# dselivanov/rsparse

Hardware: AMD Instinct MI355X
Metric: als_iterations_per_sec (higher is better)
Workload: dtype f32 (Gram products of rows > 512 / <= 32 non-zeros as 2 x fp16 / 3 x bf16 split terms of the fp32 operands, fp32 accumulate; everything else fp32); 1 GPU; WRMF implicit ALS, CG(3), synthetic 10000000x1000000, 500155883 nnz, rank 128, lambda 0.1; survey_config=3, feedback=implicit, n_items=1000000, nnz=500155883, rank=128, solver=conjugate_gradient, cg_steps=3, parallelism=rows sharded x1, factors replicated

## Files before the change

rsparse_amd/build.py:

```python
import subprocess
import sys
import time
from concurrent.futures import ThreadPoolExecutor
from pathlib import Path

PKG = Path(__file__).resolve().parent
CSRC = PKG / "csrc"
SRC = [CSRC / n for n in ("wrmf_kernels.hip", "wrmf_cgq.hip", "wrmf_cgp.hip", "wrmf_ne.hip", "wrmf_chol.hip", "wrmf_chol_wave.hip", "wrmf_chol_mf.hip", "wrmf_cg_mf.hip", "wrmf_chol_lr.hip",
                          "wrmf_topk.hip", "wrmf_topk_large.hip", "wrmf_similar.hip", "wrmf_metrics.hip", "wrmf_hits.hip", "wrmf_lists.hip", "wrmf_diversity.hip", "wrmf_mmr.hip", "wrmf_ranks.hip", "wrmf_score.hip", "wrmf_candidates.hip", "wrmf_sample.hip", "wrmf_sample_weighted.hip", "wrmf_split.hip", "wrmf_explain.hip", "wrmf_init.hip", "wrmf_ingest.hip", "wrmf_nnls.hip", "wrmf_bias.hip", "wrmf_lu.hip",
                          "wrmf_f64.hip", "wrmf_wide.hip", "wrmf_wide_cg.hip", "wrmf_ctx_kernels.hip", "wrmf_schedule.cpp", "wrmf_capi.cpp", "wrmf_f64_capi.cpp", "wrmf_ctx.cpp")]
HEADERS = [CSRC / "wrmf_chol_mf.attrs.csv", CSRC / "wrmf_mf.h", CSRC / "wrmf_internal.h", CSRC / "wrmf_capi_common.h", CSRC / "wrmf_schedule.h", CSRC / "wrmf_device.h", CSRC / "wrmf_sample_team.h", CSRC / "wrmf_wave.h", CSRC / "wrmf_ldlt.h", CSRC / "wrmf_f64.h", PKG.parent / "include" / "rsparse_wrmf_hip.h"]
DEPS = SRC + HEADERS
OUT = PKG / "lib" / "librsparse_wrmf_hip.so"
FLAGS = ["--offload-arch=gfx950", "-O3", "-std=c++17", "-fPIC"]


EXTRA_FLAGS = {n: ["-mllvm", "-forceattrs-csv-path=" + str(CSRC / "wrmf_chol_mf.attrs.csv"), "-fno-slp-vectorize"] for n in ("wrmf_chol_mf.hip", "wrmf_cg_mf.hip")}
AUDITED = {"wrmf_chol_mf.hip", "wrmf_cg_mf.hip"}
REG_LIMIT = {"wrmf_cg_mf.hip": 512}
NO_SPILL = {"wrmf_cgq.hip": ("14als_cgq_kernelILi128ELi24ELi4ELi4E",),
            "wrmf_explain.hip": ("14explain_kernelIfLi128E",),
            "wrmf_sample.hip": ("13sample_kernelILi64E", "13sample_kernelILi256E"),
            "wrmf_sample_weighted.hip": ("22sample_weighted_kernelILi64E", "22sample_weighted_kernelILi256E"),
            "wrmf_hits.hip": ("18hit_metrics_kernelILb0E", "18hit_metrics_kernelILb1E"),
            "wrmf_lists.hip": ("19list_metrics_kernelILb0E", "19list_metrics_kernelILb1E"),
            "wrmf_diversity.hip": ("21list_diversity_kernelI", "21item_inv_norms_kernelI"),
            "wrmf_mmr.hip": ("10mmr_kernelI",),
            "wrmf_split.hip": ("split_count_wave_kernel", "split_count_team_kernel", "split_write_wave_kernel", "split_write_team_kernel")}
RESOURCE_FLAG = "-Rpass-analysis=kernel-resource-usage"


def resource_violations(remarks, patterns, limit=256):
    import re
    rows, cur = [], None
    for line in remarks.splitlines():
        m = re.search(r"remark:\s+(.*?) \[-Rpass", line)
        if not m:
            continue
        t = m.group(1).strip()
        if t.startswith("Function Name:"):
            cur = {"name": t.split(":", 1)[1].strip()}
            rows.append(cur)
        elif ":" in t and cur is not None:
            k, v = t.rsplit(":", 1)
            cur[k.strip()] = v.strip()
    bad = []
    for pat in patterns:
        hit = [r for r in rows if pat in r["name"]]
        if not hit:
            bad.append((pat, "no such kernel in the compilation"))
        for r in hit:
            regs = int(r.get("VGPRs", "0")) + int(r.get("AGPRs", "0"))
            for key in ("VGPRs Spill", "ScratchSize [bytes/lane]"):
                if int(r.get(key, "0")):
                    bad.append((r["name"], "%s = %s" % (key, r[key])))
            if regs > limit:
                bad.append((r["name"], "%d vector registers" % regs))
    return bad


def audit_listing(src, extra, obj):
    sys.path.insert(0, str(PKG.parent / "tools" / "dbg"))
    import acc_audit
    lst = obj.with_suffix(".s")

    def listing(flags, floor):
        cmd = ["hipcc", *FLAGS, *flags, "-S", "--cuda-device-only", str(src), "-o", str(lst)]
        r = subprocess.run(cmd, stdout=subprocess.PIPE, stderr=subprocess.PIPE, text=True)
        if r.returncode != 0:
            raise RuntimeError("hipcc -S failed on %s:\n%s" % (src.name, r.stderr[-3000:]))
        acc, flight, _ = acc_audit.audit(str(lst), quiet=True, acc_floor=floor)
        return acc, flight, lst.read_text()
    acc, flight, text = listing(extra, 0)
    import re
    nfree = re.findall(r"\.amdhsa_kernel (\w+)[\s\S]*?\.amdhsa_next_free_vgpr (\d+)", text)
    limit = REG_LIMIT.get(src.name, 256)
    two_waves = bool(nfree) and all(int(v) <= limit for name, v in nfree if "_any" not in name)
    if acc == 0 and flight == 0 and two_waves:
        return
    print("  %s: audit of the two-waves-per-SIMD build failed (accumulator-file %d, in-flight %d, layout ok %s): rebuilding with -DMF_SAFE"
          % (src.name, acc, flight, two_waves), flush=True)
    safe = ["-DMF_SAFE"]
    cmd = ["hipcc", *FLAGS, *safe, "-c", str(src), "-o", str(obj)]
    r = subprocess.run(cmd, stdout=subprocess.PIPE, stderr=subprocess.PIPE, text=True)
    if r.returncode != 0:
        raise RuntimeError("hipcc failed on %s (MF_SAFE):\n%s" % (src.name, r.stderr[-3000:]))
    acc, flight, text = listing(safe, 96)
    if acc or flight:
        raise RuntimeError("%s: the MF_SAFE build fails the audit too (accumulator-file %d, in-flight %d)" % (src.name, acc, flight))


def build(force=False, verbose=False, out=None):
    out = Path(out) if out else OUT
    out.parent.mkdir(exist_ok=True)
    objdir = OUT.parent / "obj"
    objdir.mkdir(parents=True, exist_ok=True)
    src = [s for s in SRC if s.exists()]
    hdr_m = max(h.stat().st_mtime for h in HEADERS)
    todo, objs = [], []
    for s in src:
        o = objdir / (s.stem + ".o")
        objs.append(o)
        if force or not o.exists() or o.stat().st_mtime < max(s.stat().st_mtime, hdr_m):
            todo.append((s, o))
    if not todo and out.exists() and all(out.stat().st_mtime >= o.stat().st_mtime for o in objs):
        return out

    def compile_one(so):
        s, o = so
        t0 = time.time()
        extra = EXTRA_FLAGS.get(s.name, [])
        guard = NO_SPILL.get(s.name)
        cmd = ["hipcc", *FLAGS, *extra, *([RESOURCE_FLAG] if guard else []), "-c", str(s), "-o", str(o)]
        r = subprocess.run(cmd, stdout=subprocess.PIPE, stderr=subprocess.PIPE, text=True)
        if r.returncode != 0:
            raise RuntimeError("hipcc failed on %s:\n%s" % (s.name, r.stderr[-6000:]))
        if guard:
            bad = resource_violations(r.stderr, guard)
            if bad:
                o.unlink()
                raise RuntimeError("%s: kernels that must not spill do:\n%s" % (s.name, "\n".join("  %s: %s" % b for b in bad)))
        if s.name in AUDITED:
            audit_listing(s, extra, o)
        if verbose:
            print("  %-20s %.1f s" % (s.name, time.time() - t0), flush=True)

    with ThreadPoolExecutor(max_workers=8) as ex:
        list(ex.map(compile_one, todo))
    cmd = ["hipcc", "--offload-arch=gfx950", "-fPIC", "-shared", *map(str, objs), "-ldl", "-lpthread", "-o", str(out)]
    subprocess.check_call(cmd)
    return out


if __name__ == "__main__":
    argv = sys.argv[1:]
    outp = argv[argv.index("--out") + 1] if "--out" in argv else None
    t0 = time.time()
    print(build(force="--force" in argv, verbose=True, out=outp), "%.1f s" % (time.time() - t0))
```

rsparse_amd/csrc/wrmf_kernels.hip:

```cpp
#include "wrmf_internal.h"
#include "wrmf_device.h"

namespace rsparse_hip {
namespace {

using namespace dev;

template <int KP, int T, int W, bool IMPLICIT>
struct CgSmem {
  static constexpr int LDT = Geo<KP>::LDT;
  static constexpr size_t gram_floats = IMPLICIT ? (size_t)KP * KP : 0;
  static constexpr size_t tile_floats = (size_t)W * T * LDT;
  static constexpr size_t vec_floats = (size_t)W * KP;
  static constexpr size_t red_floats = (size_t)2 * W * KP + 2 * W;
  static constexpr size_t short_bytes = (gram_floats + tile_floats + vec_floats) * 4 + 16;
  static constexpr size_t long_bytes = (gram_floats + tile_floats + vec_floats + red_floats) * 4 + 16;
};

template <int KP, int W>
__device__ __forceinline__ void load_gram_lds(float* sG, const float* __restrict__ G, int k, int tid) {
  for (int e = tid; e < KP * KP; e += W * 64) {
    const int r = e / KP, c = e % KP;
    sG[e] = (r < k && c < k) ? G[(size_t)r * k + c] : 0.f;
  }
}

template <int KP, int T, int W, bool IMPLICIT, bool VEC>
__global__ __launch_bounds__(W * 64) void als_cg_short_kernel(AlsArgs a) {
  constexpr int EPL = Geo<KP>::EPL, LDT = Geo<KP>::LDT;
  extern __shared__ __attribute__((aligned(16))) char smem[];
  float* sG = reinterpret_cast<float*>(smem);
  float* sTiles = sG + CgSmem<KP, T, W, IMPLICIT>::gram_floats;
  float* sVecs = sTiles + CgSmem<KP, T, W, IMPLICIT>::tile_floats;
  int* sCtr = reinterpret_cast<int*>(sVecs + CgSmem<KP, T, W, IMPLICIT>::vec_floats);

  const int tid = threadIdx.x, lane = tid & 63, wv = rfl(tid >> 6);
  const int k = a.k;
  if constexpr (IMPLICIT) load_gram_lds<KP, W>(sG, a.XtX, k, tid);
  for (int e = tid; e < (int)(CgSmem<KP, T, W, IMPLICIT>::tile_floats + CgSmem<KP, T, W, IMPLICIT>::vec_floats);
       e += W * 64)
    sTiles[e] = 0.f;
  if (tid == 0) *sCtr = 0;
  __syncthreads();

  float* tile = sTiles + wv * T * LDT;
  float* vec = sVecs + wv * KP;
  const int row0 = blockIdx.x * kRowsPerWGShort;
  const int row_end = min(a.n_cols, row0 + kRowsPerWGShort);
  const int e0 = lane * EPL;
  const bool active = e0 < KP;
  const int jl = lane % T;
  double wloss = 0.0;
  const bool gb = IMPLICIT && a.gbias != 0.f;
  const float gbias = gb ? a.gbias : 0.f, ltgt = gb ? a.loss_tgt_const : 1.f;

  while (true) {
    int rr = 0;
    if (lane == 0) rr = atomicAdd(sCtr, 1);
    const int row = row0 + rfl(rr);
    if (row >= row_end) break;
    const int p1 = rfl(a.col_ptrs[row]), p2 = rfl(a.col_ptrs[row + 1]);
    const int cnt = p2 - p1;
    if (cnt > T) continue;
    float* yrow = a.Y + (size_t)row * k;
    if (cnt <= 0 && !gb) {
      for (int e = lane; e < k; e += 64) yrow[e] = 0.f;
      continue;
    }
    const bool jvalid = jl < cnt;
    const int myidx = jvalid ? a.row_idx[p1 + jl] : 0;
    const float c = jvalid ? a.vals[p1 + jl] : 0.f;
    wave_sync();
    gather_chunk<KP, T, VEC>(a.X, k, myidx, cnt, tile, lane);

    float x[EPL], r[EPL], p[EPL], ap[EPL];
#pragma unroll
    for (int u = 0; u < EPL; u++) x[u] = (active && e0 + u < k) ? yrow[e0 + u] : 0.f;
    const float lam_use =
        IMPLICIT ? 0.f : (float)(a.lambda_loss * (a.dynamic_lambda ? (double)(float)cnt : 1.0));

    put_vec<KP>(vec, x, lane, active);
    wave_sync();
    float t = tile_dot<KP, T>(tile, vec, lane);
    float wgt = jvalid ? (IMPLICIT ? c - (c - 1.f) * (t + gbias) : c - t) : 0.f;
#pragma unroll
    for (int u = 0; u < EPL; u++) r[u] = 0.f;
    tile_axpy<KP>(tile, wgt, cnt, lane, active, r);
    if constexpr (IMPLICIT) {
      gram_mv<KP>(sG, vec, 0, KP, lane, active, -1.f, r);
      if (gb) {
#pragma unroll
        for (int u = 0; u < EPL; u++) r[u] += (active && e0 + u < k) ? a.rhs_init[e0 + u] : 0.f;
      }
    } else {
#pragma unroll
      for (int u = 0; u < EPL; u++) r[u] -= lam_use * x[u];
    }
    float rs = 0.f;
#pragma unroll
    for (int u = 0; u < EPL; u++) { p[u] = r[u]; rs = fmaf(r[u], r[u], rs); }
    float rsold = wave_sum(rs);

    for (int it = 0; it < a.cg_steps; ++it) {
      wave_sync();
      put_vec<KP>(vec, p, lane, active);
      wave_sync();
      t = tile_dot<KP, T>(tile, vec, lane);
      wgt = jvalid ? (IMPLICIT ? (c - 1.f) * t : t) : 0.f;
#pragma unroll
      for (int u = 0; u < EPL; u++) ap[u] = 0.f;
      tile_axpy<KP>(tile, wgt, cnt, lane, active, ap);
      if constexpr (IMPLICIT) {
        gram_mv<KP>(sG, vec, 0, KP, lane, active, 1.f, ap);
      } else {
#pragma unroll
        for (int u = 0; u < EPL; u++) ap[u] = fmaf(lam_use, p[u], ap[u]);
      }
      float pap = 0.f;
#pragma unroll
      for (int u = 0; u < EPL; u++) pap = fmaf(p[u], ap[u], pap);
      pap = wave_sum(pap);
      const float alpha = (float)((double)rsold / (double)pap);
      rs = 0.f;
#pragma unroll
      for (int u = 0; u < EPL; u++) {
        x[u] = fmaf(alpha, p[u], x[u]);
        r[u] = fmaf(-alpha, ap[u], r[u]);
        rs = fmaf(r[u], r[u], rs);
      }
      const float rsnew = wave_sum(rs);
      if (rsnew < kCgTol) break;
      const float beta = (float)((double)rsnew / (double)rsold);
#pragma unroll
      for (int u = 0; u < EPL; u++) p[u] = fmaf(p[u], beta, r[u]);
      rsold = rsnew;
    }

    wave_sync();
    put_vec<KP>(vec, x, lane, active);
    wave_sync();
    t = tile_dot<KP, T>(tile, vec, lane);
    const float d = IMPLICIT ? ltgt - t : c - t;
    const float lj = (jvalid && lane < T) ? (IMPLICIT ? c * d * d : d * d) : 0.f;
    const float rl = wave_sum(lj);
    float xx = 0.f;
#pragma unroll
    for (int u = 0; u < EPL; u++) xx = fmaf(x[u], x[u], xx);
    xx = wave_sum(xx);
    wloss += IMPLICIT ? (double)rl + a.lambda_loss * (double)xx : (double)(rl + lam_use * xx);
#pragma unroll
    for (int u = 0; u < EPL; u++)
      if (active && e0 + u < k) yrow[e0 + u] = x[u];
  }
  if (lane == 0) a.loss_partials[(size_t)blockIdx.x * W + wv] = wloss;
}

template <int KP, int T, int W, bool IMPLICIT, bool VEC>
__global__ __launch_bounds__(W * 64) void als_cg_long_kernel(AlsArgs a, size_t loss_slot0) {
  constexpr int EPL = Geo<KP>::EPL, LDT = Geo<KP>::LDT;
  static_assert(KP % (4 * W) == 0, "Gramian k-range must split evenly over the waves");
  extern __shared__ __attribute__((aligned(16))) char smem[];
  float* sG = reinterpret_cast<float*>(smem);
  float* sTiles = sG + CgSmem<KP, T, W, IMPLICIT>::gram_floats;
  float* sVecs = sTiles + CgSmem<KP, T, W, IMPLICIT>::tile_floats;
  float* sRed = sVecs + CgSmem<KP, T, W, IMPLICIT>::vec_floats;
  float* sRedL = sRed + 2 * W * KP;

  const int tid = threadIdx.x, lane = tid & 63, wv = rfl(tid >> 6);
  const int k = a.k;
  if constexpr (IMPLICIT) load_gram_lds<KP, W>(sG, a.XtX, k, tid);
  for (int e = tid; e < (int)(CgSmem<KP, T, W, IMPLICIT>::tile_floats + CgSmem<KP, T, W, IMPLICIT>::vec_floats +
                              CgSmem<KP, T, W, IMPLICIT>::red_floats);
       e += W * 64)
    sTiles[e] = 0.f;
  __syncthreads();

  float* tile = sTiles + wv * T * LDT;
  float* vec = sVecs + wv * KP;
  const int e0 = lane * EPL;
  const bool active = e0 < KP;
  const int jl = lane % T;
  int buf = 0;
  double wloss = 0.0;
  const bool gb = IMPLICIT && a.gbias != 0.f;
  const float gbias = gb ? a.gbias : 0.f, ltgt = gb ? a.loss_tgt_const : 1.f;

  for (int li = blockIdx.x; li < a.n_long; li += gridDim.x) {
    const int row = rfl(a.long_rows[li]);
    const int p1 = rfl(a.col_ptrs[row]), p2 = rfl(a.col_ptrs[row + 1]);
    const int cnt = p2 - p1;
    const int nchunks = (cnt + T - 1) / T;
    const bool resident = nchunks <= W;
    float* yrow = a.Y + (size_t)row * k;
    const float lam_use =
        IMPLICIT ? 0.f : (float)(a.lambda_loss * (a.dynamic_lambda ? (double)(float)cnt : 1.0));

    int ccnt = 0, cidx = 0;
    float cval = 0.f;
    if (resident && wv < nchunks) {
      const int base = p1 + wv * T;
      ccnt = min(T, p2 - base);
      cidx = jl < ccnt ? a.row_idx[base + jl] : 0;
      cval = jl < ccnt ? a.vals[base + jl] : 0.f;
      wave_sync();
      gather_chunk<KP, T, VEC>(a.X, k, cidx, ccnt, tile, lane);
      wave_sync();
    }

    float x[EPL], r[EPL], p[EPL], ap[EPL];
#pragma unroll
    for (int u = 0; u < EPL; u++) x[u] = (active && e0 + u < k) ? yrow[e0 + u] : 0.f;

    auto sweep = [&](const float(&v)[EPL], const int mode, float(&out)[EPL], float& loss_out) {
      wave_sync();
      put_vec<KP>(vec, v, lane, active);
      wave_sync();
      float acc[EPL];
#pragma unroll
      for (int u = 0; u < EPL; u++) acc[u] = 0.f;
      float lacc = 0.f;
      for (int ch = wv; ch < nchunks; ch += W) {
        if (!resident) {
          const int base = p1 + ch * T;
          ccnt = min(T, p2 - base);
          cidx = jl < ccnt ? a.row_idx[base + jl] : 0;
          cval = jl < ccnt ? a.vals[base + jl] : 0.f;
          wave_sync();
          gather_chunk<KP, T, VEC>(a.X, k, cidx, ccnt, tile, lane);
          wave_sync();
        }
        const bool jvalid = jl < ccnt;
        const float t = tile_dot<KP, T>(tile, vec, lane);
        if (mode == 2) {
          const float d = IMPLICIT ? ltgt - t : cval - t;
          lacc += (jvalid && lane < T) ? (IMPLICIT ? cval * d * d : d * d) : 0.f;
        } else {
          float wgt;
          if (mode == 0) wgt = IMPLICIT ? cval - (cval - 1.f) * (t + gbias) : cval - t;
          else wgt = IMPLICIT ? (cval - 1.f) * t : t;
          wgt = jvalid ? wgt : 0.f;
          tile_axpy<KP>(tile, wgt, ccnt, lane, active, acc);
        }
      }
      float* red = sRed + buf * W * KP;
      if (mode == 2) {
        lacc = wave_sum(lacc);
        if (lane == 0) sRedL[buf * W + wv] = lacc;
      } else {
        if constexpr (IMPLICIT)
          gram_mv<KP>(sG, vec, wv * (KP / W), (wv + 1) * (KP / W), lane, active, mode == 0 ? -1.f : 1.f, acc);
        put_vec<KP>(red + wv * KP, acc, lane, active);
      }
      __syncthreads();
      if (mode == 2) {
        float s = 0.f;
#pragma unroll
        for (int w2 = 0; w2 < W; w2++) s += sRedL[buf * W + w2];
        loss_out = s;
      } else {
#pragma unroll
        for (int u = 0; u < EPL; u++) out[u] = 0.f;
#pragma unroll
        for (int w2 = 0; w2 < W; w2++) {
          if constexpr (EPL == 2) {
            const float2 q = *reinterpret_cast<const float2*>(red + w2 * KP + lane * 2);
            out[0] += q.x;
            out[1] += q.y;
          } else {
            out[0] += active ? red[w2 * KP + lane] : 0.f;
          }
        }
        if constexpr (!IMPLICIT) {
#pragma unroll
          for (int u = 0; u < EPL; u++) out[u] = fmaf(mode == 0 ? -lam_use : lam_use, v[u], out[u]);
        } else if (gb && mode == 0) {
#pragma unroll
          for (int u = 0; u < EPL; u++) out[u] += (active && e0 + u < k) ? a.rhs_init[e0 + u] : 0.f;
        }
      }
      buf ^= 1;
    };

    float dummy = 0.f;
    sweep(x, 0, r, dummy);
    float rs = 0.f;
#pragma unroll
    for (int u = 0; u < EPL; u++) { p[u] = r[u]; rs = fmaf(r[u], r[u], rs); }
    float rsold = wave_sum(rs);
    for (int it = 0; it < a.cg_steps; ++it) {
      sweep(p, 1, ap, dummy);
      float pap = 0.f;
#pragma unroll
      for (int u = 0; u < EPL; u++) pap = fmaf(p[u], ap[u], pap);
      pap = wave_sum(pap);
      const float alpha = (float)((double)rsold / (double)pap);
      rs = 0.f;
#pragma unroll
      for (int u = 0; u < EPL; u++) {
        x[u] = fmaf(alpha, p[u], x[u]);
        r[u] = fmaf(-alpha, ap[u], r[u]);
        rs = fmaf(r[u], r[u], rs);
      }
      const float rsnew = wave_sum(rs);
      if (rsnew < kCgTol) break;
      const float beta = (float)((double)rsnew / (double)rsold);
#pragma unroll
      for (int u = 0; u < EPL; u++) p[u] = fmaf(p[u], beta, r[u]);
      rsold = rsnew;
    }
    float rl = 0.f;
    sweep(x, 2, ap, rl);
    float xx = 0.f;
#pragma unroll
    for (int u = 0; u < EPL; u++) xx = fmaf(x[u], x[u], xx);
    xx = wave_sum(xx);
    if (wv == 0) {
      wloss += IMPLICIT ? (double)rl + a.lambda_loss * (double)xx : (double)(rl + lam_use * xx);
#pragma unroll
      for (int u = 0; u < EPL; u++)
        if (active && e0 + u < k) yrow[e0 + u] = x[u];
    }
  }
  if (tid == 0) a.loss_partials[loss_slot0 + blockIdx.x] = wloss;
}


template <int KP>
__global__ __launch_bounds__(256, 2) void gramian_partial_kernel(const float* __restrict__ X, int k, int64_t n,
                                                              float* __restrict__ partials,
                                                              unsigned* __restrict__ absmax_bits) {
  constexpr int NT = KP / 32, U = 4;
  const int lane = threadIdx.x & 63;
  const int64_t gw = (int64_t)blockIdx.x * 4 + (threadIdx.x >> 6), nw = (int64_t)gridDim.x * 4;
  const int col = lane & 31, half = lane >> 5;
  f32x16 acc[NT][NT];
#pragma unroll
  for (int i = 0; i < NT; i++)
#pragma unroll
    for (int j = 0; j < NT; j++)
#pragma unroll
      for (int e = 0; e < 16; e++) acc[i][j][e] = 0.f;

  float amax = 0.f;
  auto fetch = [&](const int64_t n0, float (&dst)[U][NT]) {
#pragma unroll
    for (int u = 0; u < U; u++) {
      const int64_t ent = n0 + 2 * u + half;
      const int64_t er = ent < n ? ent : n - 1;
#pragma unroll
      for (int mt = 0; mt < NT; mt++) dst[u][mt] = X[er * k + min(mt * 32 + col, k - 1)];
    }
  };
  auto take = [&](const int64_t n0, const float (&src)[U][NT], float (&dst)[U][NT]) {
#pragma unroll
    for (int u = 0; u < U; u++) {
      const bool in = n0 + 2 * u + half < n;
#pragma unroll
      for (int mt = 0; mt < NT; mt++) dst[u][mt] = src[u][mt] * ((in && mt * 32 + col < k) ? 1.f : 0.f);
    }
  };
  float av[U][NT], nx[U][NT];
  const int64_t stride = nw * 2 * U;
  int64_t n0 = gw * 2 * U;
  if (n0 < n) {
    fetch(n0, nx);
    take(n0, nx, av);
  }
  for (; n0 < n; n0 += stride) {
    const bool more = n0 + stride < n;
    if (more) fetch(n0 + stride, nx);
#pragma unroll
    for (int u = 0; u < U; u++)
#pragma unroll
      for (int mt = 0; mt < NT; mt++) amax = fmaxf(amax, fabsf(av[u][mt]));
#pragma unroll
    for (int u = 0; u < U; u++)
#pragma unroll
      for (int mt = 0; mt < NT; mt++)
#pragma unroll
        for (int nt = 0; nt <= mt; nt++)
          acc[mt][nt] = __builtin_amdgcn_mfma_f32_32x32x2f32(av[u][mt], av[u][nt], acc[mt][nt], 0, 0, 0);
    if (more) take(n0 + stride, nx, av);
  }
  if (absmax_bits) {
#pragma unroll
    for (int off = 32; off > 0; off >>= 1) amax = fmaxf(amax, __shfl_xor(amax, off));
    if (lane == 0) atomicMax(absmax_bits, __float_as_uint(amax < 3.0e38f ? amax : 3.0e38f));
  }
  float* out = partials + (size_t)gw * KP * KP;
#pragma unroll
  for (int mt = 0; mt < NT; mt++)
#pragma unroll
    for (int nt = 0; nt <= mt; nt++)
#pragma unroll
      for (int e = 0; e < 16; e++) {
        const int rr = mt * 32 + (e & 3) + 8 * (e >> 2) + 4 * half;
        out[(size_t)rr * KP + nt * 32 + col] = acc[mt][nt][e];
      }
}

__global__ void gramian_reduce_kernel(const float* __restrict__ partials, int nparts, int KP, int k, float ridge,
                                      float* __restrict__ G, double* __restrict__ diag) {
  const int e = blockIdx.x * blockDim.x + threadIdx.x;
  if (e >= k * k) return;
  const int aa = e / k, bb = e % k;
  const int ta = aa / 32, tb = bb / 32;
  const int rr = ta >= tb ? aa : bb, cc = ta >= tb ? bb : aa;
  double s = 0.0;
  const float* src = partials + (size_t)rr * KP + cc;
  for (int w = 0; w < nparts; w++) s += (double)src[(size_t)w * KP * KP];
  G[(size_t)bb * k + aa] = (float)s + (aa == bb ? ridge : 0.f);
  if (aa == bb) diag[aa] = s;
}

__global__ void trace_kernel(const double* __restrict__ diag, int k, double* __restrict__ out) {
  if (threadIdx.x == 0 && blockIdx.x == 0) {
    double s = 0.0;
    for (int i = 0; i < k; i++) s += diag[i];
    *out = s;
  }
}

__global__ __launch_bounds__(256) void weighted_sumsq_kernel(const float* __restrict__ X, int k, int64_t n,
                                                             const float* __restrict__ w, double* __restrict__ partials) {
  __shared__ double sh[4];
  const int64_t total = n * k;
  double s = 0.0;
  for (int64_t e = (int64_t)blockIdx.x * 256 + threadIdx.x; e < total; e += (int64_t)gridDim.x * 256) {
    const float v = X[e];
    const float wj = w ? w[e / k] : 1.f;
    s += (double)(v * v * wj);
  }
  for (int m = 32; m >= 1; m >>= 1) s += __shfl_xor(s, m);
  if ((threadIdx.x & 63) == 0) sh[threadIdx.x >> 6] = s;
  __syncthreads();
  if (threadIdx.x == 0) partials[blockIdx.x] = (sh[0] + sh[1]) + (sh[2] + sh[3]);
}

__global__ __launch_bounds__(256) void sum_partials_kernel(const double* __restrict__ partials, size_t n,
                                                           double* __restrict__ out) {
  __shared__ double sh[4];
  double s = 0.0;
  for (size_t e = threadIdx.x; e < n; e += 256) s += partials[e];
  for (int m = 32; m >= 1; m >>= 1) s += __shfl_xor(s, m);
  if ((threadIdx.x & 63) == 0) sh[threadIdx.x >> 6] = s;
  __syncthreads();
  if (threadIdx.x == 0) *out = (sh[0] + sh[1]) + (sh[2] + sh[3]);
}

__global__ __launch_bounds__(256) void sum_partials_stage_kernel(const double* __restrict__ partials, size_t n,
                                                                 double* __restrict__ tail) {
  __shared__ double sh[4];
  const size_t per = (n + gridDim.x - 1) / gridDim.x, lo = (size_t)blockIdx.x * per, hi = lo + per < n ? lo + per : n;
  double s = 0.0;
  for (size_t e = lo + threadIdx.x; e < hi; e += 256) s += partials[e];
  for (int m = 32; m >= 1; m >>= 1) s += __shfl_xor(s, m);
  if ((threadIdx.x & 63) == 0) sh[threadIdx.x >> 6] = s;
  __syncthreads();
  if (threadIdx.x == 0) tail[blockIdx.x] = (sh[0] + sh[1]) + (sh[2] + sh[3]);
}

__global__ void f64_to_f32_kernel(const double* __restrict__ in, float* __restrict__ out, size_t n) {
  for (size_t e = (size_t)blockIdx.x * blockDim.x + threadIdx.x; e < n; e += (size_t)gridDim.x * blockDim.x)
    out[e] = (float)in[e];
}
__global__ void f32_to_f64_kernel(const float* __restrict__ in, double* __restrict__ out, size_t n) {
  for (size_t e = (size_t)blockIdx.x * blockDim.x + threadIdx.x; e < n; e += (size_t)gridDim.x * blockDim.x)
    out[e] = (double)in[e];
}

template <typename K>
hipError_t set_lds(K kernel, size_t bytes) {
  return hipFuncSetAttribute(reinterpret_cast<const void*>(kernel), hipFuncAttributeMaxDynamicSharedMemorySize,
                             (int)bytes);
}

template <int KP, bool IMPLICIT, bool VEC>
hipError_t launch_cg_t(const AlsArgs& a, hipStream_t s, hipEvent_t* ev) {
  constexpr int T = kTileNnz, W = kWavesPerWG;
  using SM = CgSmem<KP, T, W, IMPLICIT>;
  hipError_t err;
  const int grid_s = (a.n_cols + kRowsPerWGShort - 1) / kRowsPerWGShort;
  if (ev && (err = hipEventRecord(ev[0], s)) != hipSuccess) return err;
  if (grid_s > 0) {
    auto ks = als_cg_short_kernel<KP, T, W, IMPLICIT, VEC>;
    if ((err = set_lds(ks, SM::short_bytes)) != hipSuccess) return err;
    prof_note(ev, reinterpret_cast<const void*>(ks));
    hipLaunchKernelGGL(ks, dim3(grid_s), dim3(W * 64), SM::short_bytes, s, a);
    if ((err = hipGetLastError()) != hipSuccess) return err;
  }
  if (ev && (err = hipEventRecord(ev[1], s)) != hipSuccess) return err;
  if (a.n_long > 0) {
    const int grid_l = (a.n_long + kRowsPerWGLong - 1) / kRowsPerWGLong;
    auto kl = als_cg_long_kernel<KP, T, W, IMPLICIT, VEC>;
    if ((err = set_lds(kl, SM::long_bytes)) != hipSuccess) return err;
    prof_note(ev ? ev + 1 : nullptr, reinterpret_cast<const void*>(kl));
    hipLaunchKernelGGL(kl, dim3(grid_l), dim3(W * 64), SM::long_bytes, s, a, (size_t)grid_s * W);
    if ((err = hipGetLastError()) != hipSuccess) return err;
  }
  if (ev && (err = hipEventRecord(ev[2], s)) != hipSuccess) return err;
  return hipSuccess;
}

}

int padded_rank(int k) {
  if (k <= 0) return 0;
  if (k <= 32) return 32;
  if (k <= 64) return 64;
  if (k <= 128) return 128;
  return 0;
}

size_t cg_loss_slots(int n_cols, int n_long) {
  const size_t grid_s = ((size_t)n_cols + kRowsPerWGShort - 1) / kRowsPerWGShort;
  const size_t grid_l = ((size_t)n_long + kRowsPerWGLong - 1) / kRowsPerWGLong;
  return grid_s * kWavesPerWG + grid_l;
}

size_t chol_loss_slots(int n_cols) {
  return (size_t)(n_cols < kCholMaxGrid ? (n_cols > 0 ? n_cols : 1) : kCholMaxGrid);
}

hipError_t launch_als_cg(const AlsArgs& a, bool implicit, hipStream_t s, hipEvent_t* ev) {
  const int KP = padded_rank(a.k);
  const bool vec = (a.k % 4 == 0) && ((reinterpret_cast<uintptr_t>(a.X) & 15) == 0);
#define RSP_DISPATCH(KPV)                                                             \
  if (KP == KPV) {                                                                    \
    if (implicit) return vec ? launch_cg_t<KPV, true, true>(a, s, ev) : launch_cg_t<KPV, true, false>(a, s, ev); \
    return vec ? launch_cg_t<KPV, false, true>(a, s, ev) : launch_cg_t<KPV, false, false>(a, s, ev);             \
  }
  RSP_DISPATCH(32)
  RSP_DISPATCH(64)
  RSP_DISPATCH(128)
#undef RSP_DISPATCH
  return hipErrorInvalidValue;
}

hipError_t launch_sum_partials(const double* partials, size_t n, double* out, hipStream_t s, double* tail) {
  if (tail && n > 16384) {
    hipLaunchKernelGGL(sum_partials_stage_kernel, dim3(kSumStageBlocks), dim3(256), 0, s, partials, n, tail);
    hipError_t err = hipGetLastError();
    if (err != hipSuccess) return err;
    hipLaunchKernelGGL(sum_partials_kernel, dim3(1), dim3(256), 0, s, tail, (size_t)kSumStageBlocks, out);
    return hipGetLastError();
  }
  hipLaunchKernelGGL(sum_partials_kernel, dim3(1), dim3(256), 0, s, partials, n, out);
  return hipGetLastError();
}

static int gramian_waves(int64_t n) {
  int64_t w = (n + 63) / 64;
  if (w < 1) w = 1;
  if (w > 1024) w = 1024;
  return (int)((w + 3) / 4 * 4);
}

size_t gramian_scratch_floats(int k, int64_t n) {
  const int KP = padded_rank(k);
  return (size_t)gramian_waves(n) * KP * KP + 2 * 128  + 16;
}

hipError_t launch_gramian(const float* X, int k, int64_t n, float ridge, float* XtX, double* sumsq,
                          float* scratch, hipStream_t s, hipEvent_t* ev, unsigned* absmax_bits) {
  const int KP = padded_rank(k);
  if (!KP) return hipErrorInvalidValue;
  const int waves = gramian_waves(n);
  float* partials = scratch;
  double* diag = reinterpret_cast<double*>(scratch + (((size_t)waves * KP * KP + 1) & ~(size_t)1));
  const int grid = waves / 4;
  if (ev) (void)hipEventRecord(ev[0], s);
  prof_note(ev, KP == 32 ? reinterpret_cast<const void*>(gramian_partial_kernel<32>)
                         : (KP == 64 ? reinterpret_cast<const void*>(gramian_partial_kernel<64>)
                                     : reinterpret_cast<const void*>(gramian_partial_kernel<128>)));
  prof_note(ev ? ev + 1 : nullptr, reinterpret_cast<const void*>(gramian_reduce_kernel));
  if (KP == 32) hipLaunchKernelGGL(gramian_partial_kernel<32>, dim3(grid), dim3(256), 0, s, X, k, n, partials, absmax_bits);
  else if (KP == 64) hipLaunchKernelGGL(gramian_partial_kernel<64>, dim3(grid), dim3(256), 0, s, X, k, n, partials, absmax_bits);
  else hipLaunchKernelGGL(gramian_partial_kernel<128>, dim3(grid), dim3(256), 0, s, X, k, n, partials, absmax_bits);
  hipError_t err = hipGetLastError();
  if (err != hipSuccess) return err;
  if (ev) (void)hipEventRecord(ev[1], s);
  hipLaunchKernelGGL(gramian_reduce_kernel, dim3((k * k + 255) / 256), dim3(256), 0, s, partials, waves, KP, k,
                     ridge, XtX, diag);
  if ((err = hipGetLastError()) != hipSuccess) return err;
  if (sumsq) {
    hipLaunchKernelGGL(trace_kernel, dim3(1), dim3(64), 0, s, diag, k, sumsq);
    err = hipGetLastError();
  }
  if (ev) (void)hipEventRecord(ev[2], s);
  return err;
}

hipError_t launch_weighted_sumsq(const float* X, int k, int64_t n, const float* w, double* out, double* scratch,
                                 hipStream_t s) {
  int64_t blocks = (n * k + 256 * 16 - 1) / (256 * 16);
  if (blocks < 1) blocks = 1;
  if (blocks > 1024) blocks = 1024;
  hipLaunchKernelGGL(weighted_sumsq_kernel, dim3((int)blocks), dim3(256), 0, s, X, k, n, w, scratch);
  hipError_t err = hipGetLastError();
  if (err != hipSuccess) return err;
  return launch_sum_partials(scratch, (size_t)blocks, out, s);
}

hipError_t launch_f64_to_f32(const double* in, float* out, size_t n, hipStream_t s) {
  if (!n) return hipSuccess;
  size_t blocks = (n + 1023) / 1024;
  if (blocks > 4096) blocks = 4096;
  hipLaunchKernelGGL(f64_to_f32_kernel, dim3((int)blocks), dim3(256), 0, s, in, out, n);
  return hipGetLastError();
}
hipError_t launch_f32_to_f64(const float* in, double* out, size_t n, hipStream_t s) {
  if (!n) return hipSuccess;
  size_t blocks = (n + 1023) / 1024;
  if (blocks > 4096) blocks = 4096;
  hipLaunchKernelGGL(f32_to_f64_kernel, dim3((int)blocks), dim3(256), 0, s, in, out, n);
  return hipGetLastError();
}

}
```

Before: 8.634 iterations/s.

## Deepen gramian prefetch pipeline and split partial reduction into parallel slices

The gramian partial kernel now prefetches two row batches ahead with sched barriers around the loads, uses 32-bit byte offsets from a clamped base pointer, and folds the absmax update into the take step. The single reduce over up to 1024 wave partials per element is split into a 16-slice parallel stage in double precision followed by a short final reduce. The aim is to hide global-load latency in the MFMA loop and to parallelise the serial reduction. In exchange it holds more live registers (a new no-spill guard is added), adds a kernel launch, and needs extra scratch for the slices.

```diff
diff --git a/rsparse_amd/build.py b/rsparse_amd/build.py
--- a/rsparse_amd/build.py
+++ b/rsparse_amd/build.py
@@ -19,6 +19,7 @@
 AUDITED = {"wrmf_chol_mf.hip", "wrmf_cg_mf.hip"}
 REG_LIMIT = {"wrmf_cg_mf.hip": 512}
 NO_SPILL = {"wrmf_cgq.hip": ("14als_cgq_kernelILi128ELi24ELi4ELi4E",),
+            "wrmf_kernels.hip": ("22gramian_partial_kernelILi128E",),
             "wrmf_explain.hip": ("14explain_kernelIfLi128E",),
             "wrmf_sample.hip": ("13sample_kernelILi64E", "13sample_kernelILi256E"),
             "wrmf_sample_weighted.hip": ("22sample_weighted_kernelILi64E", "22sample_weighted_kernelILi256E"),
diff --git a/rsparse_amd/csrc/wrmf_kernels.hip b/rsparse_amd/csrc/wrmf_kernels.hip
--- a/rsparse_amd/csrc/wrmf_kernels.hip
+++ b/rsparse_amd/csrc/wrmf_kernels.hip
@@ -325,13 +325,16 @@
 }
 
 
+constexpr int kGramAhead = 2;
+constexpr int kGramSlices = 16;
+
 template <int KP>
 __global__ __launch_bounds__(256, 2) void gramian_partial_kernel(const float* __restrict__ X, int k, int64_t n,
                                                               float* __restrict__ partials,
                                                               unsigned* __restrict__ absmax_bits) {
-  constexpr int NT = KP / 32, U = 4;
+  constexpr int NT = KP / 32, U = 4, D = kGramAhead;
   const int lane = threadIdx.x & 63;
-  const int64_t gw = (int64_t)blockIdx.x * 4 + (threadIdx.x >> 6), nw = (int64_t)gridDim.x * 4;
+  const int64_t gw = (int64_t)blockIdx.x * 4 + __builtin_amdgcn_readfirstlane(threadIdx.x >> 6), nw = (int64_t)gridDim.x * 4;
   const int col = lane & 31, half = lane >> 5;
   f32x16 acc[NT][NT];
 #pragma unroll
@@ -342,13 +345,18 @@
       for (int e = 0; e < 16; e++) acc[i][j][e] = 0.f;
 
   float amax = 0.f;
+  unsigned cofs[NT];
+#pragma unroll
+  for (int mt = 0; mt < NT; mt++) cofs[mt] = 4u * (unsigned)min(mt * 32 + col, k - 1);
   auto fetch = [&](const int64_t n0, float (&dst)[U][NT]) {
+    const int64_t c0 = n0 < n ? n0 : n - 1;
+    const int last = (int)(n - 1 - c0 < 2 * U - 1 ? n - 1 - c0 : 2 * U - 1);
+    const char* base = reinterpret_cast<const char*>(X + c0 * k);
 #pragma unroll
     for (int u = 0; u < U; u++) {
-      const int64_t ent = n0 + 2 * u + half;
-      const int64_t er = ent < n ? ent : n - 1;
-#pragma unroll
-      for (int mt = 0; mt < NT; mt++) dst[u][mt] = X[er * k + min(mt * 32 + col, k - 1)];
+      const unsigned rofs = 4u * (unsigned)k * (unsigned)min(2 * u + half, last);
+#pragma unroll
+      for (int mt = 0; mt < NT; mt++) dst[u][mt] = *reinterpret_cast<const float*>(base + (rofs + cofs[mt]));
     }
   };
   auto take = [&](const int64_t n0, const float (&src)[U][NT], float (&dst)[U][NT]) {
@@ -356,31 +364,46 @@
     for (int u = 0; u < U; u++) {
       const bool in = n0 + 2 * u + half < n;
 #pragma unroll
-      for (int mt = 0; mt < NT; mt++) dst[u][mt] = src[u][mt] * ((in && mt * 32 + col < k) ? 1.f : 0.f);
+      for (int mt = 0; mt < NT; mt++) {
+        dst[u][mt] = src[u][mt] * ((in && mt * 32 + col < k) ? 1.f : 0.f);
+        amax = fmaxf(amax, fabsf(dst[u][mt]));
+      }
     }
   };
-  float av[U][NT], nx[U][NT];
+  float av[U][NT], nx[D][U][NT];
+  auto multiply = [&]() {
+#pragma unroll
+    for (int u = 0; u < U; u++)
+#pragma unroll
+      for (int mt = 0; mt < NT; mt++)
+#pragma unroll
+        for (int nt = 0; nt <= mt; nt++)
+          acc[mt][nt] = __builtin_amdgcn_mfma_f32_32x32x2f32(av[u][mt], av[u][nt], acc[mt][nt], 0, 0, 0);
+  };
   const int64_t stride = nw * 2 * U;
   int64_t n0 = gw * 2 * U;
   if (n0 < n) {
-    fetch(n0, nx);
-    take(n0, nx, av);
-  }
-  for (; n0 < n; n0 += stride) {
-    const bool more = n0 + stride < n;
-    if (more) fetch(n0 + stride, nx);
-#pragma unroll
-    for (int u = 0; u < U; u++)
-#pragma unroll
-      for (int mt = 0; mt < NT; mt++) amax = fmaxf(amax, fabsf(av[u][mt]));
-#pragma unroll
-    for (int u = 0; u < U; u++)
-#pragma unroll
-      for (int mt = 0; mt < NT; mt++)
-#pragma unroll
-        for (int nt = 0; nt <= mt; nt++)
-          acc[mt][nt] = __builtin_amdgcn_mfma_f32_32x32x2f32(av[u][mt], av[u][nt], acc[mt][nt], 0, 0, 0);
-    if (more) take(n0 + stride, nx, av);
+#pragma unroll
+    for (int d = 0; d < D; d++) fetch(n0 + d * stride, nx[d]);
+    take(n0, nx[0], av);
+    while (n0 + D * stride < n) {
+#pragma unroll
+      for (int b = 0; b < D; b++) {
+        __builtin_amdgcn_sched_barrier(0);
+        fetch(n0 + D * stride, nx[b]);
+        __builtin_amdgcn_sched_barrier(0);
+        multiply();
+        n0 += stride;
+        take(n0, nx[(b + 1) % D], av);
+      }
+    }
+#pragma unroll
+    for (int b = 0; b < D; b++) {
+      multiply();
+      n0 += stride;
+      if (n0 >= n) break;
+      take(n0, nx[(b + 1) % D], av);
+    }
   }
   if (absmax_bits) {
 #pragma unroll
@@ -399,7 +422,20 @@
       }
 }
 
-__global__ void gramian_reduce_kernel(const float* __restrict__ partials, int nparts, int KP, int k, float ridge,
+__global__ __launch_bounds__(256) void gramian_slice_kernel(const float* __restrict__ partials, int nparts, int KP, int k,
+                                                            double* __restrict__ slices) {
+  const int p = blockIdx.x * 256 + threadIdx.x;
+  const int rr = p / KP, cc = p % KP;
+  if (rr / 32 < cc / 32 || rr >= k || cc >= k) return;
+  const int lo = (int)((int64_t)blockIdx.y * nparts / kGramSlices), hi = (int)((int64_t)(blockIdx.y + 1) * nparts / kGramSlices);
+  double s = 0.0;
+  const float* src = partials + p;
+#pragma unroll 8
+  for (int w = lo; w < hi; w++) s += (double)src[(size_t)w * KP * KP];
+  slices[(size_t)blockIdx.y * KP * KP + p] = s;
+}
+
+__global__ void gramian_reduce_kernel(const double* __restrict__ slices, int KP, int k, float ridge,
                                       float* __restrict__ G, double* __restrict__ diag) {
   const int e = blockIdx.x * blockDim.x + threadIdx.x;
   if (e >= k * k) return;
@@ -407,8 +443,9 @@
   const int ta = aa / 32, tb = bb / 32;
   const int rr = ta >= tb ? aa : bb, cc = ta >= tb ? bb : aa;
   double s = 0.0;
-  const float* src = partials + (size_t)rr * KP + cc;
-  for (int w = 0; w < nparts; w++) s += (double)src[(size_t)w * KP * KP];
+  const double* src = slices + (size_t)rr * KP + cc;
+#pragma unroll
+  for (int y = 0; y < kGramSlices; y++) s += src[(size_t)y * KP * KP];
   G[(size_t)bb * k + aa] = (float)s + (aa == bb ? ridge : 0.f);
   if (aa == bb) diag[aa] = s;
 }
@@ -558,7 +595,8 @@
 
 size_t gramian_scratch_floats(int k, int64_t n) {
   const int KP = padded_rank(k);
-  return (size_t)gramian_waves(n) * KP * KP + 2 * 128  + 16;
+  return (size_t)gramian_waves(n) * KP * KP + 2 * 128  + 16 +
+         2 * (size_t)kGramSlices * KP * KP ;
 }
 
 hipError_t launch_gramian(const float* X, int k, int64_t n, float ridge, float* XtX, double* sumsq,
@@ -568,6 +606,7 @@
   const int waves = gramian_waves(n);
   float* partials = scratch;
   double* diag = reinterpret_cast<double*>(scratch + (((size_t)waves * KP * KP + 1) & ~(size_t)1));
+  double* slices = diag + 128;
   const int grid = waves / 4;
   if (ev) (void)hipEventRecord(ev[0], s);
   prof_note(ev, KP == 32 ? reinterpret_cast<const void*>(gramian_partial_kernel<32>)
@@ -580,8 +619,9 @@
   hipError_t err = hipGetLastError();
   if (err != hipSuccess) return err;
   if (ev) (void)hipEventRecord(ev[1], s);
-  hipLaunchKernelGGL(gramian_reduce_kernel, dim3((k * k + 255) / 256), dim3(256), 0, s, partials, waves, KP, k,
-                     ridge, XtX, diag);
+  hipLaunchKernelGGL(gramian_slice_kernel, dim3(KP * KP / 256, kGramSlices), dim3(256), 0, s, partials, waves, KP, k, slices);
+  if ((err = hipGetLastError()) != hipSuccess) return err;
+  hipLaunchKernelGGL(gramian_reduce_kernel, dim3((k * k + 255) / 256), dim3(256), 0, s, slices, KP, k, ridge, XtX, diag);
   if ((err = hipGetLastError()) != hipSuccess) return err;
   if (sumsq) {
     hipLaunchKernelGGL(trace_kernel, dim3(1), dim3(64), 0, s, diag, k, sumsq);
```

New measurement: 8.716 iterations/s (median of 6 runs). About the same (+1.0%).
